# dangeross/rust-bitcoinconsensus

Hardware: AMD Instinct MI355X
Metric: ECDSA verifies/sec (node) at 1/2/4/8 MI355X; % of int-ALU roofline (higher is better)
Workload: dtype u32; 1 GPU; C2: synthetic P2WPKH inputs, BIP143 sighash + ECDSA verify (BASELINE.json configs[1]); inputs_per_gpu=1000000, global_inputs=1000000, parallelism=shard x1 (independent tuples, no collective)

## Files before the change

### rust-bitcoinconsensus_amd/csrc/ecdsa_lane.h

```cpp
#pragma once
#include "secp256k1_device.h"
#include "sha256_device.h"

namespace bcc {

#ifndef BCC_WQ_BITS
#define BCC_WQ_BITS 4
#endif
constexpr int WQ = BCC_WQ_BITS;
#ifndef BCC_WG_BITS
#define BCC_WG_BITS 10
#endif
constexpr int WG = BCC_WG_BITS;
constexpr int QTAB = 1 << (WQ - 1);
constexpr int GTAB = 1 << (WG - 1);
constexpr int TOPQ = (127 / WQ) * WQ;
static_assert(TOPQ + WQ >= 128, "top Q digit must cover bit 127");
constexpr int TOPG = (127 / WG) * WG;
static_assert(TOPG + WG >= 128 && TOPG <= TOPQ, "top G digit must cover bit 127 inside the ladder");

BCC_HD u32 bits_at(u32 l0, u32 l1, u32 l2, u32 l3, int pos, int w) {
    int li = pos >> 5, sh = pos & 31;
    u32 a = li == 0 ? l0 : li == 1 ? l1 : li == 2 ? l2 : l3;
    u32 b = li == 0 ? l1 : li == 1 ? l2 : li == 2 ? l3 : 0u;
    u32 v = sh ? ((a >> sh) | (b << (32 - sh))) : a;
    return v & ((1u << w) - 1u);
}

BCC_HD u32 digit_index(u32 l0, u32 l1, u32 l2, u32 l3, int pos, int w, int top, bool& neg) {
    u32 v = bits_at(l0, l1, l2, l3, pos + 1, w);
    if (pos == top) {
        neg = false;
        return v;
    }
    u32 half = 1u << (w - 1), mask = half - 1u;
    bool positive = (v & half) != 0;
    neg = !positive;
    return positive ? (v & mask) : (~v & mask);
}

struct QTableArray {
    fe e[QTAB][3];
    BCC_HD void put(int i, int f, const fe& a) { e[i][f] = a; }
    BCC_HD void get(int i, int f, fe& a) const { a = e[i][f]; }
    BCC_HD void get_pair(int i, int which, fe& x, fe& y) const {
        x = e[i][which];
        y = e[i][2];
    }
};

struct GTableArray {
    const fe* xy;
    BCC_HD void get(int tab, int i, fe& x, fe& y) const {
        x = xy[(tab * GTAB + i) * 2 + 0];
        y = xy[(tab * GTAB + i) * 2 + 1];
    }
};

BCC_HD void acc_add(gej& acc, bool& inf, const fe& px, const fe& py, const fe& sigma,
                    bool use_zinv) {
    if (inf) {
        if (use_zinv) {
            fe s2, s3;
            fe_sqr(s2, sigma);
            fe_mul(s3, s2, sigma);
            fe_mul(acc.x, px, s2);
            fe_mul(acc.y, py, s3);
        } else {
            acc.x = px;
            acc.y = py;
        }
        acc.z = fe_one();
        inf = false;
        return;
    }
    gej r;
    bool rinf;
    gej_add_zinv(r, rinf, acc, px, py, sigma, use_zinv);
    acc = r;
    inf = rinf;
}

enum : u32 {
    LS_VALID = 1u, LS_NEG0 = 2u, LS_NEG1 = 4u, LS_CORR0 = 8u,
};

template <class QT>
BCC_HD void build_q_table_coz(const fe& qx, const fe& qy, QT& qt, fe& sigma) {
    fe dx, dy, tx, ty;
    {
        fe b, e, l, sx, m, t;
        fe_sqr(b, qx);
        fe_sqr(e, qy);
        fe_sqr(l, e);
        fe_add(t, qx, e);
        fe_sqr(t, t);
        fe_sub(t, t, b);
        fe_sub(t, t, l);
        fe_shl<1>(sx, t);
        fe_shl<1>(m, b);
        fe_add(m, m, b);
        fe_sqr(t, m);
        fe_shl<1>(dx, sx);
        fe_sub(dx, t, dx);
        fe_sub(t, sx, dx);
        fe_mul(t, m, t);
        fe_shl<3>(ty, l);
        fe_sub(dy, t, ty);
        tx = sx;
    }
    qt.put(0, 0, tx);
    qt.put(0, 2, ty);
    for (int i = 1; i < QTAB; i++) {
        fe h, c, w1, w2, d, a1, t, ry;
        fe_sub(h, dx, tx);
        fe_sqr(c, h);
        fe_mul(w1, dx, c);
        fe_mul(w2, tx, c);
        fe_sub(ry, dy, ty);
        fe_sqr(d, ry);
        fe_sub(t, w1, w2);
        fe_mul(a1, dy, t);
        fe_sub(t, d, w1);
        fe_sub(tx, t, w2);
        fe_sub(t, w1, tx);
        fe_mul(t, ry, t);
        fe_sub(ty, t, a1);
        dx = w1;
        dy = a1;
        qt.put(i, 0, tx);
        qt.put(i, 2, ty);
        qt.put(i, 1, h);
    }
    fe f = fe_one(), f2, f3, beta;
    {
        const u32 bl[8] = BCC_BETA_LIMBS;
        fe_set(beta, bl);
    }
    for (int i = QTAB - 1; i >= 0; i--) {
        fe ex, ey, h;
        qt.get(i, 0, ex);
        qt.get(i, 2, ey);
        if (i > 0) qt.get(i, 1, h);
        if (i < QTAB - 1) {
            fe_sqr(f2, f);
            fe_mul(f3, f2, f);
            fe_mul(ex, ex, f2);
            fe_mul(ey, ey, f3);
        }
        fe bx;
        fe_mul(bx, ex, beta);
        qt.put(i, 0, ex);
        qt.put(i, 1, bx);
        qt.put(i, 2, ey);
        if (i > 0) fe_mul(f, f, h);
    }
    fe y2;
    fe_shl<1>(y2, qy);
    fe_mul(sigma, f, y2);
}

BCC_HD void curve_rhs(fe& r, const fe& x) {
    fe seven = fe_const(7, 0, 0, 0, 0, 0, 0, 0);
    fe_sqr(r, x);
    fe_mul(r, r, x);
    fe_add(r, r, seven);
}


BCC_HD void schnorr_challenge(sc& e, const fe& rx, const fe& px, const sc& m) {
    const u32 N[8] = BCC_N_LIMBS;
    u32 s[8] = {0x9cecba11u, 0x23925381u, 0x11679112u, 0xd1627e0fu,
                0x97c87550u, 0x003cc765u, 0x90f61164u, 0x33e9b66au};
    u32 w[16];
#pragma unroll
    for (int j = 0; j < 8; j++) {
        w[j] = rx.v[7 - j];
        w[8 + j] = px.v[7 - j];
    }
    sha256_compress(s, w);
#pragma unroll
    for (int j = 0; j < 8; j++) w[j] = m.v[7 - j];
    w[8] = 0x80000000u;
#pragma unroll
    for (int j = 9; j < 15; j++) w[j] = 0;
    w[15] = 160 * 8;
    sha256_compress(s, w);
#pragma unroll
    for (int i = 0; i < 8; i++) e.v[i] = s[7 - i];
    if (!u256_lt(e.v, N)) {
        u32 tmp[8];
        u256_sub(tmp, e.v, N);
        for (int i = 0; i < 8; i++) e.v[i] = tmp[i];
    }
}

BCC_HD bool schnorr_y_even(const fe& ye, const fe& zinv) {
    fe z2, z3, y;
    fe_sqr(z2, zinv);
    fe_mul(z3, z2, zinv);
    fe_mul(y, ye, z3);
    fe_normalize(y);
    return (y.v[0] & 1u) == 0;
}

template <class GT>
BCC_HD bool ecmult_gen_lane(const sc& k_in, fe& xo, fe& yo, const GT& gt) {
    if (sc_is_zero(k_in)) return false;
    u32 c0 = k_in.v[0], c1 = k_in.v[1], c2 = k_in.v[2], c3 = k_in.v[3];
    u32 d0 = k_in.v[4], d1 = k_in.v[5], d2 = k_in.v[6], d3 = k_in.v[7];
    bool corr2 = (c0 & 1u) == 0, corr3 = (d0 & 1u) == 0;
    c0 |= 1u;
    d0 |= 1u;
    fe one = fe_one();
    gej acc;
    bool inf = false;
    {
        bool ng;
        u32 idx = digit_index(c0, c1, c2, c3, TOPG, WG, TOPG, ng);
        gt.get(0, (int)idx, acc.x, acc.y);
        acc.z = one;
    }
    for (int pos = TOPG; pos >= 0; pos--) {
        if (pos != TOPG && !inf) {
            gej t;
            gej_double(t, acc);
            acc = t;
        }
        if (pos % WG) continue;
        for (int slot = 2; slot < 4; slot++) {
            if (slot == 2 && pos == TOPG) continue;
            bool dneg;
            u32 idx = slot == 2 ? digit_index(c0, c1, c2, c3, pos, WG, TOPG, dneg)
                                : digit_index(d0, d1, d2, d3, pos, WG, TOPG, dneg);
            fe px, py;
            gt.get(slot - 2, (int)idx, px, py);
            if (dneg) fe_neg(py, py);
// ... 117 lines not shown
```

### rust-bitcoinconsensus_amd/csrc/ecdsa_twist.h

```cpp
#pragma once
#include <stddef.h>

#include <algorithm>
#include <thread>
#include <vector>

#include "ecdsa_lane.h"

namespace bcc {

#ifndef BCC_COMB_BITS
#define BCC_COMB_BITS 16
#endif
constexpr int WC = BCC_COMB_BITS;
constexpr int CTAB = 1 << (WC - 1);
constexpr int CTOP = (256 + WC - 1) / WC - 1;
constexpr int CWIN = CTOP + 1;
static_assert(WC * CTOP + 1 + (WC - 1) >= 256, "top comb digit must cover bit 255");

enum : u32 {
    LS_NEGU1 = 1u << 7,
    LS_U1ZERO = 1u << 8,
    LS_COMP = 1u << 9,
    LS_PAR = 1u << 10,
// ... 69 lines not shown
    build_q_table_coz(qx, qy, qt, st.sigma);
    st.flags = flags;
    return true;
}

BCC_HD bool twist_prep_u2(u32 flags, const sc& r_in, const sc& s_in, const sc* sinv_pre,
                          TwistState& st, sc* sinv_out = nullptr) {
    const u32 N[8] = BCC_N_LIMBS;
    st.flags = 0;
    if (!(flags & LS_VALID)) return false;
    if (u256_is_zero(r_in.v) || u256_is_zero(s_in.v)) return false;
    if (!u256_lt(r_in.v, N) || !u256_lt(s_in.v, N)) return false;
    sc sinv, u2, k1, k2;
    if (sinv_pre) sinv = *sinv_pre;
    else sc_inv(sinv, s_in);
    if (sinv_out) *sinv_out = sinv;
    sc_mul(u2, r_in, sinv);
    sc_split_lambda(k1, k2, u2);
    if ((k1.v[4] | k1.v[5] | k1.v[6] | k1.v[7]) != 0) {
        sc_neg(k1, k1);
        flags |= LS_NEG0;
    }
    if ((k2.v[4] | k2.v[5] | k2.v[6] | k2.v[7]) != 0) {
        sc_neg(k2, k2);
        flags |= LS_NEG1;
    }
    for (int i = 0; i < 4; i++) {
        st.k[0][i] = k1.v[i];
        st.k[1][i] = k2.v[i];
    }
    for (int s = 0; s < 2; s++) {
        if ((st.k[s][0] & 1u) == 0) flags |= LS_CORR0 << s;
        st.k[s][0] |= 1u;
    }
    st.flags = flags;
    st.r = r_in;
    return true;
}

BCC_HD void twist_prep_u1(const sc& m_in, const sc& sinv, u32* flags, u32 (&k2)[4], u32 (&k3)[4]) {
    const u32 N[8] = BCC_N_LIMBS;
    sc m = m_in, u1;
    if (!u256_lt(m.v, N)) {
        u32 tmp[8];
        u256_sub(tmp, m.v, N);
        for (int i = 0; i < 8; i++) m.v[i] = tmp[i];
    }
    sc_mul(u1, m, sinv);
    if (sc_is_zero(u1)) {
        *flags |= LS_U1ZERO;
        u1.v[0] = 1u;
    } else if ((u1.v[0] & 1u) == 0) {
        sc_neg(u1, u1);
        *flags |= LS_NEGU1;
    }
    for (int i = 0; i < 4; i++) {
        k2[i] = u1.v[i];
        k3[i] = u1.v[4 + i];
    }
}

BCC_HD bool twist_prep_scalars(u32 flags, const sc& r_in, const sc& s_in, const sc& m_in,
                               const sc* sinv_pre, TwistState& st) {
    sc sinv;
    if (!twist_prep_u2(flags, r_in, s_in, sinv_pre, st, &sinv)) return false;
    twist_prep_u1(m_in, sinv, &st.flags, st.k[2], st.k[3]);
    return true;
}

template <class QT>
BCC_HD bool twist_prep_lane(u32 tag, const fe& px, const fe& py, const sc& r_in, const sc& s_in,
                            const sc& m_in, const sc* sinv_pre, QT& qt, TwistState& st) {
    if (!twist_prep_key(tag, px, py, qt, st)) return false;
    return twist_prep_scalars(st.flags, r_in, s_in, m_in, sinv_pre, st);
}

template <class ST, class QT>
BCC_HD bool twist_accumulate_q(const ST& st, const QT& qt, gej& acc) {
    const bool neg0 = (st.flags & LS_NEG0) != 0, neg1 = (st.flags & LS_NEG1) != 0;
    const fe one = fe_one();
    bool inf = false;
    {
        bool ng;
        u32 idx = digit_index(st.kword(0, 0), st.kword(0, 1), st.kword(0, 2), st.kword(0, 3), TOPQ,
                              WQ, TOPQ, ng);
        qt.get((int)idx, 0, acc.x);
        qt.get((int)idx, 2, acc.y);
        if (neg0) fe_neg(acc.y, acc.y);
        acc.z = one;
    }
#pragma unroll 1
    for (int pos = TOPQ; pos >= -1; pos--) {
        if (pos >= 0 && pos != TOPQ && !inf) {
            gej t;
            gej_double(t, acc);
            acc = t;
        }
        if (pos >= 0 && (pos % WQ) != 0) continue;
#pragma unroll 1
        for (int slot = 0; slot < 2; slot++) {
            const bool kneg = slot == 0 ? neg0 : neg1;
            u32 idx;
            bool sneg;
            if (pos >= 0) {
                if (slot == 0 && pos == TOPQ) continue;
                bool dneg;
                idx = digit_index(st.kword(slot, 0), st.kword(slot, 1), st.kword(slot, 2),
                                  st.kword(slot, 3), pos, WQ, TOPQ, dneg);
                sneg = dneg ^ kneg;
            } else {
                if (!(st.flags & (LS_CORR0 << slot))) continue;
                idx = 0;
                sneg = !kneg;
            }
            fe px, py;
            qt.get_pair((int)idx, slot, px, py);
            if (sneg) fe_neg(py, py);
            acc_add(acc, inf, px, py, one, false);
        }
    }
    return inf;
}

template <class ST, class QT>
BCC_HD bool twist_accumulate_q_half(const ST& st, const QT& qt, gej& acc, int slot) {
    const bool kneg = (st.flags & (slot == 0 ? LS_NEG0 : LS_NEG1)) != 0;
    const fe one = fe_one();
    bool inf = false;
    {
        bool ng;
        const u32 idx = digit_index(st.kword(slot, 0), st.kword(slot, 1), st.kword(slot, 2),
                                    st.kword(slot, 3), TOPQ, WQ, TOPQ, ng);
        qt.get_pair((int)idx, slot, acc.x, acc.y);
        if (kneg) fe_neg(acc.y, acc.y);
        acc.z = one;
    }
#pragma unroll 1
    for (int pos = TOPQ; pos >= -1; pos--) {
        if (pos >= 0 && pos != TOPQ && !inf) {
            gej t;
            gej_double(t, acc);
            acc = t;
        }
        if (pos >= 0 && ((pos % WQ) != 0 || pos == TOPQ)) continue;
        u32 idx;
        bool sneg;
        if (pos >= 0) {
            bool dneg;
            idx = digit_index(st.kword(slot, 0), st.kword(slot, 1), st.kword(slot, 2),
                              st.kword(slot, 3), pos, WQ, TOPQ, dneg);
            sneg = dneg ^ kneg;
        } else {
            if (!(st.flags & (LS_CORR0 << slot))) continue;
            idx = 0;
            sneg = !kneg;
        }
        fe px, py;
        qt.get_pair((int)idx, slot, px, py);
        if (sneg) fe_neg(py, py);
        acc_add(acc, inf, px, py, one, false);
    }
    return inf;
}

template <class ST, class GC>
BCC_HD bool twist_accumulate_g(const ST& st, const GC& gc, gej& acc) {
    const fe one = fe_one();
    bool inf = false;
    {
        bool ng;
        u32 idx = comb_digit(st, WC * CTOP, ng);
        gc.get(CTOP, (int)idx, acc.x, acc.y);
        acc.z = one;
    }
#pragma unroll 1
    for (int win = CTOP - 1; win >= 0; win--) {
        bool neg;
        u32 idx = comb_digit(st, WC * win, neg);
        fe px, py;
        gc.get(win, (int)idx, px, py);
        if (neg) fe_neg(py, py);
        acc_add(acc, inf, px, py, one, false);
    }
    if (st.flags & LS_NEGU1) fe_neg(acc.y, acc.y);
    if (st.flags & LS_U1ZERO) inf = true;
    return inf;
}

BCC_HD bool twist_combine(const gej& A, const gej& B, const fe& sigma, const fe& v, const sc& r,
                          fe& al, fe& be, fe& K) {
    fe zb, zb2, z12, u1, u2, s1, s2, h, hh, t;
    fe_mul(zb, B.z, sigma);
    fe_sqr(zb2, zb);
    fe_sqr(z12, A.z);
    fe_mul(u2, B.x, z12);
    fe_mul(t, z12, A.z);
    fe_mul(s2, B.y, t);
    fe_mul(t, A.y, zb2);
    fe_mul(t, t, zb);
    fe_mul(s1, t, v);
    fe_mul(t, A.x, zb2);
    fe_mul(u1, t, v);
    fe_sub(h, u2, u1);
    if (fe_is_zero(h)) return false;
    fe_mul(be, s2, s1);
    fe_shl<1>(be, be);
    if (fe_is_zero(be)) return false;
    fe_sqr(hh, h);
    fe_mul(t, z12, zb2);
    fe_mul(t, t, v);
    fe_mul(K, t, hh);
    fe xr;
    for (int i = 0; i < 8; i++) xr.v[i] = r.v[i];
    fe_mul(al, xr, K);
    fe_sqr(t, s2);
    fe_sub(al, al, t);
    fe_sqr(t, s1);
    fe_mul(t, t, v);
    fe_sub(al, al, t);
    fe_mul(t, hh, h);
    fe_add(al, al, t);
    fe_mul(t, u1, hh);
    fe_shl<1>(t, t);
    fe_add(al, al, t);
    return true;
}

BCC_HD bool twist_is_key_y(const fe& al, const fe& binv, const fe& v, const fe& ychk, u32 flags) {
    fe g, g2;
    fe_mul(g, al, binv);
    fe_neg(g, g);
    fe_normalize(g);
    fe_sqr(g2, g);
    if (!fe_equal(g2, v)) return false;
    if (flags & LS_COMP) return (g.v[0] & 1u) == ((flags & LS_PAR) ? 1u : 0u);
    return fe_equal(g, ychk);
}

BCC_HD int twist_final(const fe& al, const fe& K, const fe& binv, const fe& v, const fe& ychk,
                       u32 flags, const sc& r) {
    if (twist_is_key_y(al, binv, v, ychk, flags)) return 1;
    const u32 PMN[8] = BCC_PMN_LIMBS;
    if (!u256_lt(r.v, PMN)) return 0;
    const u32 N[8] = BCC_N_LIMBS;
    fe nf, t, al2;
    fe_set(nf, N);
    fe_mul(t, K, nf);
    fe_add(al2, al, t);
    return twist_is_key_y(al2, binv, v, ychk, flags) ? 1 : 0;
}

BCC_HD void gej_add_gej(gej& r, bool& inf, const gej& a, const gej& b) {
    fe z22, z12, u1, u2, s1, s2, h, rr, hh, hhh, v, t;
    fe_sqr(z22, b.z);
    fe_sqr(z12, a.z);
    fe_mul(u1, a.x, z22);
    fe_mul(u2, b.x, z12);
    fe_mul(s1, a.y, z22);
    fe_mul(s1, s1, b.z);
    fe_mul(s2, b.y, z12);
    fe_mul(s2, s2, a.z);
    fe_sub(h, u2, u1);
    fe_sub(rr, s2, s1);
    if (fe_is_zero(h)) {
        if (fe_is_zero(rr)) {
            gej_double(r, a);
            inf = false;
        } else {
            inf = true;
            r = a;
        }
        return;
    }
    fe_sqr(hh, h);
    fe_mul(hhh, h, hh);
    fe_mul(v, u1, hh);
    fe_mul(t, a.z, b.z);
    fe_mul(r.z, t, h);
    fe_sqr(t, rr);
    fe_sub(t, t, hhh);
    fe_sub(t, t, v);
    fe_sub(r.x, t, v);
    fe_sub(t, v, r.x);
    fe_mul(t, rr, t);
    fe_mul(hhh, s1, hhh);
    fe_sub(r.y, t, hhh);
    inf = false;
}

BCC_HD int twist_exceptional(const gej& A, bool ainf, const gej& B, bool binf, const fe& sigma,
                             const fe& v, const fe& ychk, u32 flags, const sc& r) {
    const u32 N[8] = BCC_N_LIMBS;
    fe w;
    if (flags & LS_COMP) {
        if (!fe_sqrt(w, v)) return 0;
        fe_normalize(w);
        if ((w.v[0] & 1u) != ((flags & LS_PAR) ? 1u : 0u)) fe_neg(w, w);
    } else {
        w = ychk;
    }
    if (ainf && binf) return 0;
    gej be = B, R;
    bool rinf = false;
    fe zb;
    fe_mul(zb, B.z, sigma);
    fe_mul(be.z, zb, w);
    if (binf) R = A;
    else if (ainf) R = be;
    else gej_add_gej(R, rinf, A, be);
    if (rinf) return 0;
    fe z2, lhs, xr;
    fe_sqr(z2, R.z);
    for (int i = 0; i < 8; i++) xr.v[i] = r.v[i];
    fe_mul(lhs, xr, z2);
    if (fe_equal(lhs, R.x)) return 1;
    const u32 PMN[8] = BCC_PMN_LIMBS;
    if (!u256_lt(r.v, PMN)) return 0;
    u32 xn[8];
    u256_add(xn, r.v, N);
    for (int i = 0; i < 8; i++) xr.v[i] = xn[i];
    fe_mul(lhs, xr, z2);
    return fe_equal(lhs, R.x) ? 1 : 0;
}

enum : u32 { TW_REJECT = 0, TW_NORMAL = 1, TW_EXCEPT = 2 };

template <class QT, class GC>
BCC_HD int ecdsa_verify_twist_lane(u32 tag, const fe& px, const fe& py, const sc& r,
                                   const sc& s, const sc& m, QT& qt, const GC& gc) {
    TwistState st;
    if (!twist_prep_lane(tag, px, py, r, s, m, nullptr, qt, st)) return 0;
    gej A, B;
    const bool binf = twist_accumulate_q(st, qt, B);
    const bool ainf = twist_accumulate_g(st, gc, A);
    fe al, be, K;
    if (binf || ainf || !twist_combine(A, B, st.sigma, st.v, st.r, al, be, K))
        return twist_exceptional(A, ainf, B, binf, st.sigma, st.v, st.ychk, st.flags, st.r);
    fe binv;
    fe_inv(binv, be);
    return twist_final(al, K, binv, st.v, st.ychk, st.flags, st.r);
}

#if !defined(__HIP_DEVICE_COMPILE__)
inline int wnaf5_128(int8_t (&d)[132], const u32 (&k)[4]) {
    typedef unsigned __int128 u128;
    u128 lo = (u128)((uint64_t)k[2] | (uint64_t)k[3] << 32) << 64 | ((uint64_t)k[0] | (uint64_t)k[1] << 32);
    uint64_t hi = 0;
    int n = 0;
    while (lo | hi) {
        int v = 0;
        if (lo & 1) {
            v = (int)(lo & 31);
            if (v >= 16) v -= 32;
            if (v > 0) {
                lo -= (u128)v;
            } else {
                const u128 o = lo;
                lo += (u128)(-v);
                if (lo < o) hi++;
            }
        }
        d[n++] = (int8_t)v;
        lo = lo >> 1 | (u128)(hi & 1) << 127;
        hi >>= 1;
    }
    return n;
}

template <class ST, class QT>
inline bool twist_accumulate_q_wnaf(const ST& st, const u32 (&k1)[4], const u32 (&k2)[4], const QT& qt,
                                    gej& acc) {
    int8_t d[2][132];
    const int n0 = wnaf5_128(d[0], k1), n1 = wnaf5_128(d[1], k2);
    const bool kneg[2] = {(st.flags & LS_NEG0) != 0, (st.flags & LS_NEG1) != 0};
    const fe one = fe_one();
    bool inf = true;
    acc.x = acc.y = fe_zero();
    acc.z = one;
    for (int i = std::max(n0, n1) - 1; i >= 0; i--) {
        if (!inf) {
            gej t;
            gej_double(t, acc);
            acc = t;
        }
        for (int slot = 0; slot < 2; slot++) {
            const int v = i < (slot ? n1 : n0) ? d[slot][i] : 0;
            if (v == 0) continue;
            fe px, py;
            qt.get_pair((v < 0 ? -v : v) >> 1, slot, px, py);
            if ((v < 0) != kneg[slot]) fe_neg(py, py);
            acc_add(acc, inf, px, py, one, false);
        }
    }
    return inf;
}

template <class QT, class GC>
inline int ecdsa_verify_twist_host(u32 tag, const fe& px, const fe& py, const sc& r, const sc& s,
                                   const sc& m, QT& qt, const GC& gc) {
    TwistState st;
    if (!twist_prep_key(tag, px, py, qt, st)) return 0;
    sc sinv;
    if (!twist_prep_u2(st.flags, r, s, nullptr, st, &sinv)) return 0;
    u32 k1[4], k2[4];
    for (int i = 0; i < 4; i++) {
        k1[i] = st.k[0][i];
        k2[i] = st.k[1][i];
    }
    if (st.flags & LS_CORR0) k1[0] &= ~1u;
    if (st.flags & (LS_CORR0 << 1)) k2[0] &= ~1u;
    twist_prep_u1(m, sinv, &st.flags, st.k[2], st.k[3]);
    gej A, B;
    const bool binf = twist_accumulate_q_wnaf(st, k1, k2, qt, B);
    const bool ainf = twist_accumulate_g(st, gc, A);
    fe al, be, K;
    if (binf || ainf || !twist_combine(A, B, st.sigma, st.v, st.r, al, be, K))
        return twist_exceptional(A, ainf, B, binf, st.sigma, st.v, st.ychk, st.flags, st.r);
    fe binv;
    fe_inv(binv, be);
    return twist_final(al, K, binv, st.v, st.ychk, st.flags, st.r);
}
#endif


template <class QT>
BCC_HD bool schnorr_twist_prep(const fe& px, const fe& rx, const sc& s_in, const sc& m, QT& qt,
                               TwistState& st) {
    const u32 N[8] = BCC_N_LIMBS;
    st.flags = 0;
    if (!fe_lt_p(rx)) return false;
    if (!u256_lt(s_in.v, N)) return false;
    if (!fe_lt_p(px)) return false;
    fe v;
    curve_rhs(v, px);
    sc e, u2, u1 = s_in, k1, k2;
    schnorr_challenge(e, rx, px, m);
    sc_neg(u2, e);
    u32 flags = LS_VALID | LS_COMP;
    sc_split_lambda(k1, k2, u2);
    if ((k1.v[4] | k1.v[5] | k1.v[6] | k1.v[7]) != 0) {
        sc_neg(k1, k1);
        flags |= LS_NEG0;
    }
    if ((k2.v[4] | k2.v[5] | k2.v[6] | k2.v[7]) != 0) {
        sc_neg(k2, k2);
        flags |= LS_NEG1;
    }
    if (sc_is_zero(u1)) {
        flags |= LS_U1ZERO;
        u1.v[0] = 1u;
    } else if ((u1.v[0] & 1u) == 0) {
        sc_neg(u1, u1);
        flags |= LS_NEGU1;
    }
    for (int i = 0; i < 4; i++) {
        st.k[0][i] = k1.v[i];
        st.k[1][i] = k2.v[i];
        st.k[2][i] = u1.v[i];
        st.k[3][i] = u1.v[4 + i];
    }
    for (int q = 0; q < 2; q++) {
        if ((st.k[q][0] & 1u) == 0) flags |= LS_CORR0 << q;
        st.k[q][0] |= 1u;
    }
    st.flags = flags;
    for (int i = 0; i < 8; i++) st.r.v[i] = rx.v[i];
    st.v = v;
    st.ychk = fe_zero();
    fe qx, qy;
    fe_mul(qx, px, v);
    fe_sqr(qy, v);
    build_q_table_coz(qx, qy, qt, st.sigma);
    return true;
}

BCC_HD bool schnorr_twist_combine(const gej& A, const gej& B, const fe& sigma, const fe& v,
                                  const fe& rx, fe& al, fe& be, fe& dd, fe& c0, fe& c1) {
    fe zb, zb2, z12, u1, u2, s1, s2, h, hh, t, x3r, m;
    fe_mul(zb, B.z, sigma);
    fe_sqr(zb2, zb);
    fe_sqr(z12, A.z);
    fe_mul(u2, B.x, z12);
    fe_mul(t, z12, A.z);
    fe_mul(s2, B.y, t);
    fe_mul(t, A.y, zb2);
    fe_mul(t, t, zb);
    fe_mul(s1, t, v);
    fe_mul(t, A.x, zb2);
    fe_mul(u1, t, v);
    fe_sub(h, u2, u1);
    if (fe_is_zero(h)) return false;
    fe_mul(be, s2, s1);
    fe_shl<1>(be, be);
    if (fe_is_zero(be)) return false;
    fe_mul(t, A.z, zb);
    fe_mul(t, t, h);
    fe_sqr(dd, t);
// ... 155 lines not shown
```

### rust-bitcoinconsensus_amd/csrc/ecdsa_verify.hip

```cpp
#include <atomic>
#include <cstdio>
#include <cstdlib>
#include <memory>
#include <string>

#include "bcc_amd.h"
#include "ecdsa_lane.h"
#include "ecdsa_twist.h"
#include "gpu_common.h"
#include "host/devices.h"
#include "host/host_verify.h"
#include "host/taproot_host.h"
#include "pipeline.h"

namespace bcc {

constexpr size_t LANE_STRIDE = 64;
__device__ __forceinline__ u32* lane_words(u32* base, size_t t, int W) {
    return base + (t >> 6) * (size_t)(W * 64) + (t & 63);
}
__device__ __forceinline__ const u32* lane_words(const u32* base, size_t t, int W) {
    return base + (t >> 6) * (size_t)(W * 64) + (t & 63);
}

struct QTableGlobal {
    u32* base;
    __device__ static int field_off(int f) { return f == 0 ? 0 : f == 1 ? 16 : 8; }
    __device__ void put(int i, int f, const fe& a) {
        uint4* p = reinterpret_cast<uint4*>(base + i * 32 + field_off(f));
        p[0] = make_uint4(a.v[0], a.v[1], a.v[2], a.v[3]);
        p[1] = make_uint4(a.v[4], a.v[5], a.v[6], a.v[7]);
        if (f == 2) {
            uint4* q = reinterpret_cast<uint4*>(base + i * 32 + 24);
            q[0] = p[0];
            q[1] = p[1];
        }
    }
    __device__ void get(int i, int f, fe& a) const {
        const uint4* p = reinterpret_cast<const uint4*>(base + i * 32 + field_off(f));
        const uint4 u = p[0], v = p[1];
        a.v[0] = u.x; a.v[1] = u.y; a.v[2] = u.z; a.v[3] = u.w;
        a.v[4] = v.x; a.v[5] = v.y; a.v[6] = v.z; a.v[7] = v.w;
    }
    __device__ void get_pair(int i, int which, fe& x, fe& y) const {
        const uint4* p = reinterpret_cast<const uint4*>(base + i * 32 + 16 * which);
        const uint4 a = p[0], b = p[1], c = p[2], d = p[3];
        x.v[0] = a.x; x.v[1] = a.y; x.v[2] = a.z; x.v[3] = a.w;
        x.v[4] = b.x; x.v[5] = b.y; x.v[6] = b.z; x.v[7] = b.w;
        y.v[0] = c.x; y.v[1] = c.y; y.v[2] = c.z; y.v[3] = c.w;
        y.v[4] = d.x; y.v[5] = d.y; y.v[6] = d.z; y.v[7] = d.w;
    }
};
__device__ __forceinline__ u32* lane_table(u32* qtab, size_t t);
constexpr int QTABLE_WORDS = QTAB * 32;
__device__ __forceinline__ u32* lane_table(u32* qtab, size_t t) { return qtab + t * QTABLE_WORDS; }
constexpr int PRE_WORDS = 8;

__device__ __forceinline__ void load_be32(fe& r, const uint8_t* p) {
    const uint4* q = reinterpret_cast<const uint4*>(p);
    uint4 a = q[0], b = q[1];
    u32 w[8] = {a.x, a.y, a.z, a.w, b.x, b.y, b.z, b.w};
    fe_from_be_words(r, w);
}
__device__ __forceinline__ void load_be32(sc& r, const uint8_t* p) {
    fe t;
    load_be32(t, p);
#pragma unroll
    for (int k = 0; k < 8; k++) r.v[k] = t.v[k];
}
__device__ __forceinline__ void load_limbs(sc& r, const u32* p) {
    const uint4* q = reinterpret_cast<const uint4*>(p);
    uint4 a = q[0], b = q[1];
    r.v[0] = a.x; r.v[1] = a.y; r.v[2] = a.z; r.v[3] = a.w;
    r.v[4] = b.x; r.v[5] = b.y; r.v[6] = b.z; r.v[7] = b.w;
}
__device__ __forceinline__ void store_limbs(u32* p, const sc& a) {
    uint4* q = reinterpret_cast<uint4*>(p);
    q[0] = make_uint4(a.v[0], a.v[1], a.v[2], a.v[3]);
    q[1] = make_uint4(a.v[4], a.v[5], a.v[6], a.v[7]);
}

__device__ __forceinline__ void sanitize_s(sc& s) {
    const u32 N[8] = BCC_N_LIMBS;
    if (u256_is_zero(s.v) || !u256_lt(s.v, N)) {
        s.v[0] = 1;
#pragma unroll
        for (int k = 1; k < 8; k++) s.v[k] = 0;
    }
}

#ifndef BCC_INV_PER_THREAD
#define BCC_INV_PER_THREAD 16
#endif
#ifndef BCC_FIN_PER_THREAD
#define BCC_FIN_PER_THREAD 16
#endif
constexpr size_t INV_PER_THREAD = BCC_INV_PER_THREAD;
constexpr size_t FIN_PER_THREAD = BCC_FIN_PER_THREAD;

__global__ __launch_bounds__(256) void batch_sinv_kernel(const uint8_t* __restrict__ ps,
                                                         u32* __restrict__ sinv, size_t n,
                                                         size_t T) {
    const size_t t = (size_t)blockIdx.x * blockDim.x + threadIdx.x;
    if (t >= n || t >= T) return;
    sc acc, s;
    size_t last = t;
    load_be32(acc, ps + 32 * t);
    sanitize_s(acc);
    store_limbs(sinv + 8 * t, acc);
    for (size_t i = t + T; i < n; i += T) {
        load_be32(s, ps + 32 * i);
        sanitize_s(s);
        sc_mul(acc, acc, s);
        store_limbs(sinv + 8 * i, acc);
        last = i;
    }
    sc inv;
    sc_inv(inv, acc);
    for (size_t i = last; i >= t + T; i -= T) {
        load_be32(s, ps + 32 * i);
        sanitize_s(s);
        sc prev, out;
        load_limbs(prev, sinv + 8 * (i - T));
        sc_mul(out, inv, prev);
        sc_mul(inv, inv, s);
        store_limbs(sinv + 8 * i, out);
    }
    store_limbs(sinv + 8 * t, inv);
}
// ... 44 lines not shown
};

struct GCombGlobal {
    const u32* base;
    __device__ void get(int win, int i, fe& x, fe& y) const {
        const uint4* q = reinterpret_cast<const uint4*>(base + ((size_t)win * CTAB + i) * 16);
        const uint4 a = q[0], b = q[1], c = q[2], d = q[3];
        x.v[0] = a.x; x.v[1] = a.y; x.v[2] = a.z; x.v[3] = a.w;
        x.v[4] = b.x; x.v[5] = b.y; x.v[6] = b.z; x.v[7] = b.w;
        y.v[0] = c.x; y.v[1] = c.y; y.v[2] = c.z; y.v[3] = c.w;
        y.v[4] = d.x; y.v[5] = d.y; y.v[6] = d.z; y.v[7] = d.w;
    }
};

__device__ __forceinline__ void park_gej(u32* q, const gej& a, bool inf) {
    uint4* p = reinterpret_cast<uint4*>(q);
    p[0] = make_uint4(a.x.v[0], a.x.v[1], a.x.v[2], a.x.v[3]);
    p[1] = make_uint4(a.x.v[4], a.x.v[5], a.x.v[6], a.x.v[7]);
    p[2] = make_uint4(a.y.v[0], a.y.v[1], a.y.v[2], a.y.v[3]);
    p[3] = make_uint4(a.y.v[4], a.y.v[5], a.y.v[6], a.y.v[7]);
    p[4] = make_uint4(a.z.v[0], a.z.v[1], a.z.v[2], a.z.v[3]);
    p[5] = make_uint4(a.z.v[4], a.z.v[5], a.z.v[6], a.z.v[7]);
    p[6] = make_uint4(inf ? 1u : 0u, 0u, 0u, 0u);
}
__device__ __forceinline__ bool unpark_gej(const u32* q, gej& a) {
    asm volatile("" : "+v"(q));
    const uint4* p = reinterpret_cast<const uint4*>(q);
    uint4 u;
    u = p[0]; a.x.v[0] = u.x; a.x.v[1] = u.y; a.x.v[2] = u.z; a.x.v[3] = u.w;
    u = p[1]; a.x.v[4] = u.x; a.x.v[5] = u.y; a.x.v[6] = u.z; a.x.v[7] = u.w;
    u = p[2]; a.y.v[0] = u.x; a.y.v[1] = u.y; a.y.v[2] = u.z; a.y.v[3] = u.w;
    u = p[3]; a.y.v[4] = u.x; a.y.v[5] = u.y; a.y.v[6] = u.z; a.y.v[7] = u.w;
    u = p[4]; a.z.v[0] = u.x; a.z.v[1] = u.y; a.z.v[2] = u.z; a.z.v[3] = u.w;
    u = p[5]; a.z.v[4] = u.x; a.z.v[5] = u.y; a.z.v[6] = u.z; a.z.v[7] = u.w;
    return p[6].x != 0;
}
constexpr int PARK_B = 0, PARK_A = 32;

__global__ __launch_bounds__(256) __attribute__((amdgpu_waves_per_eu(3, 3))) void ecdsa_tprep_kernel(
    const uint8_t* __restrict__ tag, const uint8_t* __restrict__ px,
    const uint8_t* __restrict__ py, const uint8_t* __restrict__ pr, const uint8_t* __restrict__ ps,
    const uint8_t* __restrict__ pm, const u32* __restrict__ psinv, size_t base, size_t cnt,
    u32* __restrict__ qtab, u32* __restrict__ state) {
    const size_t t = (size_t)blockIdx.x * blockDim.x + threadIdx.x;
    if (t >= cnt) return;
    const size_t i = base + t;
    fe x, y;
    sc r, s, m, si;
    load_be32(x, px + 32 * i);
    load_be32(y, py + 32 * i);
    load_be32(r, pr + 32 * i);
    load_be32(s, ps + 32 * i);
    load_be32(m, pm + 32 * i);
    load_limbs(si, psinv + 8 * i);
    QTableGlobal qt{lane_table(qtab, t)};
    TwistState st;
    twist_prep_lane(tag[i], x, y, r, s, m, &si, qt, st);
    u32* w = lane_words(state, t, TSTATE_WORDS);
#pragma unroll
    for (int a = 0; a < 4; a++)
#pragma unroll
        for (int b = 0; b < 4; b++) w[(T_K + a * 4 + b) * LANE_STRIDE] = st.k[a][b];
    w[T_FLAGS * LANE_STRIDE] = st.flags;
    tw_store(w, T_SIGMA, st.sigma.v);
    tw_store(w, T_R, st.r.v);
    tw_store(w, T_V, st.v.v);
    tw_store(w, T_Y, st.ychk.v);
}

#ifndef BCC_TLADDER_WG
#define BCC_TLADDER_WG 256
#endif
constexpr int TLADDER_WG = BCC_TLADDER_WG;

__device__ __forceinline__ void twist_q_part(u32* lt, const TwistStateView& st) {
    gej B;
    const bool binf = twist_accumulate_q(st, QTableGlobal{lt}, B);
    park_gej(lt + PARK_B, B, binf);
}

template <bool BIP340>
__device__ __forceinline__ void twist_g_part(u32* w, u32* lt, const u32* gcomb, TwistStateView& st) {
    u32 stat = TW_NORMAL;
    gej A, B;
    const bool ainf = twist_accumulate_g(st, GCombGlobal{gcomb}, A);
    const bool binf = unpark_gej(lt + PARK_B, B);
    fe v, al, be, K;
    sc r;
    st.get_v(v);
    st.get_r(r);
    bool ok;
    if constexpr (BIP340) {
        fe c0, c1, rx;
#pragma unroll
        for (int j = 0; j < 8; j++) rx.v[j] = r.v[j];
        ok = !binf && !ainf && schnorr_twist_combine(A, B, st.sigma, v, rx, al, be, K, c0, c1);
        if (ok) {
            tw_store(w, T_C0, c0.v);
            tw_store(w, T_C1, c1.v);
        }
    } else {
        ok = !binf && !ainf && twist_combine(A, B, st.sigma, v, r, al, be, K);
    }
    if (!ok) {
        park_gej(lt + PARK_A, A, ainf);
        stat = TW_EXCEPT;
    } else {
        tw_store(w, T_AL, al.v);
        tw_store(w, T_BE, be.v);
        tw_store(w, T_KK, K.v);
    }
    w[T_STAT * LANE_STRIDE] = stat;
}

template <bool BIP340>
__global__ __launch_bounds__(TLADDER_WG) __attribute__((amdgpu_waves_per_eu(BCC_LADDER_WAVES, BCC_LADDER_WAVES))) void twist_ladder_kernel(
    u32* __restrict__ state, u32* __restrict__ qtab, const u32* __restrict__ gcomb, size_t cnt) {
    const size_t t = (size_t)blockIdx.x * blockDim.x + threadIdx.x;
    if (t >= cnt) return;
    u32* w = lane_words(state, t, TSTATE_WORDS);
    TwistStateView st;
    st.p = w;
    st.flags = w[T_FLAGS * LANE_STRIDE];
    if (!(st.flags & LS_VALID)) {
        w[T_STAT * LANE_STRIDE] = TW_REJECT;
        return;
    }
    tw_load(st.sigma.v, w, T_SIGMA);
    u32* lt = lane_table(qtab, t);
    twist_q_part(lt, st);
    twist_g_part<BIP340>(w, lt, gcomb, st);
}

__global__ __launch_bounds__(TLADDER_WG) __attribute__((amdgpu_waves_per_eu(BCC_LADDER_WAVES, BCC_LADDER_WAVES))) void schnorr_tladder_kernel(
    const uint8_t* __restrict__ psig, const uint8_t* __restrict__ pm,
    const uint8_t* __restrict__ ppk, size_t base, size_t cnt, u32* __restrict__ qtab,
    u32* __restrict__ state, const u32* __restrict__ gcomb) {
    const size_t t = (size_t)blockIdx.x * blockDim.x + threadIdx.x;
    if (t >= cnt) return;
    const size_t i = base + t;
    u32* w = lane_words(state, t, TSTATE_WORDS);
    u32* lt = lane_table(qtab, t);
    {
        fe px, rx;
        sc s, m;
        load_be32(rx, psig + 64 * i);
        load_be32(s, psig + 64 * i + 32);
        load_be32(m, pm + 32 * i);
        load_be32(px, ppk + 32 * i);
        QTableGlobal qt{lt};
        TwistState st;
        schnorr_twist_prep(px, rx, s, m, qt, st);
#pragma unroll
        for (int a = 0; a < 4; a++)
#pragma unroll
            for (int b = 0; b < 4; b++) w[(T_K + a * 4 + b) * LANE_STRIDE] = st.k[a][b];
        w[T_FLAGS * LANE_STRIDE] = st.flags;
        tw_store(w, T_SIGMA, st.sigma.v);
        tw_store(w, T_R, st.r.v);
        tw_store(w, T_V, st.v.v);
        tw_store(w, T_Y, st.ychk.v);
    }
    TwistStateView sv;
    sv.p = w;
    sv.flags = w[T_FLAGS * LANE_STRIDE];
    if (!(sv.flags & LS_VALID)) {
        w[T_STAT * LANE_STRIDE] = TW_REJECT;
        return;
    }
    tw_load(sv.sigma.v, w, T_SIGMA);
    twist_q_part(lt, sv);
    twist_g_part<true>(w, lt, gcomb, sv);
}

#ifndef BCC_LADDERQ_WAVES
#define BCC_LADDERQ_WAVES BCC_LADDER_WAVES
#endif
__global__ __launch_bounds__(TLADDER_WG) __attribute__((amdgpu_waves_per_eu(BCC_LADDERQ_WAVES, BCC_LADDERQ_WAVES))) void twist_keyq_kernel(
    const uint8_t* __restrict__ tag, const uint8_t* __restrict__ px, const uint8_t* __restrict__ py,
    const uint8_t* __restrict__ pr, const uint8_t* __restrict__ ps, const u32* __restrict__ psinv,
    size_t cnt, u32* __restrict__ qtab, u32* __restrict__ state, const u32* __restrict__ emap,
    size_t ecount, size_t base) {
    const size_t t = base + (size_t)blockIdx.x * blockDim.x + threadIdx.x;
    if (t >= cnt) return;
    if (emap && emap[t] < ecount) return;
    u32* w = lane_words(state, t, TSTATE_WORDS);
    u32* lt = lane_table(qtab, t);
    {
// ... 828 lines not shown
```

### rust-bitcoinconsensus_amd/csrc/secp256k1_device.h

```cpp
#pragma once
#include <stdint.h>
#include <string.h>

#if defined(__HIPCC__)
#include <hip/hip_runtime.h>
#include "fe_asm.h"
#include "fe_asm_gen.h"
#define BCC_HD __host__ __device__ __attribute__((always_inline)) inline
#define BCC_HD_NOINLINE __host__ __device__ __attribute__((noinline))
#else
#define BCC_HD inline
#define BCC_HD_NOINLINE
#endif

#include "modinv_device.h"

namespace bcc {

typedef uint32_t u32;
typedef uint64_t u64;

struct fe {
    u32 v[8];
};
// ... 697 lines not shown
    {
        const u32 a[8] = BCC_MB1_LIMBS, b[8] = BCC_MB2_LIMBS, l[8] = BCC_LAMBDA_LIMBS;
#pragma unroll
        for (int i = 0; i < 8; i++) {
            mb1.v[i] = a[i];
            mb2.v[i] = b[i];
            lam.v[i] = l[i];
        }
    }
    sc_mul_shift_384(c1, k, G1);
    sc_mul_shift_384(c2, k, G2);
    sc_mul(c1, c1, mb1);
    sc_mul(c2, c2, mb2);
    sc_add(k2, c1, c2);
    sc_mul(k1, k2, lam);
    sc_neg(k1, k1);
    sc_add(k1, k1, k);
}

struct gej {
    fe x, y, z;
};

BCC_HD void gej_double(gej& r, const gej& a) {
    fe A, B, C, D, E, F, t;
    fe_sqr(A, a.x);
    fe_sqr(B, a.y);
    fe_sqr(C, B);
    fe_add(t, a.x, B);
    fe_sqr(t, t);
    fe_sub(t, t, A);
    fe_sub(t, t, C);
    fe_shl<1>(D, t);
    fe_shl<1>(E, A);
    fe_add(E, E, A);
    fe_sqr(F, E);
    fe_mul(r.z, a.y, a.z);
    fe_shl<1>(r.z, r.z);
    fe_shl<1>(t, D);
    fe_sub(r.x, F, t);
    fe_sub(t, D, r.x);
    fe_mul(t, E, t);
    fe_shl<3>(C, C);
    fe_sub(r.y, t, C);
}

BCC_HD void gej_add_zinv(gej& r, bool& inf, const gej& a, const fe& bx, const fe& by,
                         const fe& bzinv, bool use_zinv, fe* hout = nullptr) {
    fe az, z12, u2, s2, h, rr, hh, hhh, v, t;
    if (use_zinv) fe_mul(az, a.z, bzinv);
    else az = a.z;
    fe_sqr(z12, az);
    fe_mul(u2, bx, z12);
    fe_mul(s2, by, z12);
    fe_mul(s2, s2, az);
    fe_sub(h, u2, a.x);
    fe_sub(rr, s2, a.y);
    if (fe_is_zero(h)) {
        if (fe_is_zero(rr)) {
            gej_double(r, a);
            inf = false;
        } else {
            inf = true;
            r = a;
        }
        return;
    }
    if (hout) *hout = h;
    fe_sqr(hh, h);
    fe_mul(hhh, h, hh);
    fe_mul(v, a.x, hh);
    fe_mul(r.z, a.z, h);
    fe_sqr(t, rr);
    fe_sub(t, t, hhh);
    fe_sub(t, t, v);
    fe_sub(r.x, t, v);
    fe_sub(t, v, r.x);
    fe_mul(t, rr, t);
    fe_mul(hhh, a.y, hhh);
    fe_sub(r.y, t, hhh);
    inf = false;
}

}
```

Baseline: 115.1 million verifies/s.

## Use XYZZ coordinates for G comb, precompute negated Q-table y, merge first adds

The generator comb accumulation moves from Jacobian to XYZZ coordinates, so each mixed add needs fewer squarings and the final combine reuses ZZ and ZZZ directly. The Q table now stores a negated y entry, so lookups pick the sign by address instead of calling fe_neg on the loaded value. The first two digits of both ladders are merged with a cheaper affine plus affine add, which skips one generic add and one doubling iteration. In exchange each point carries an extra field element, which raises register pressure and state size, and the exceptional path pays a conversion back to Jacobian.

```diff
diff --git a/rust-bitcoinconsensus_amd/csrc/ecdsa_lane.h b/rust-bitcoinconsensus_amd/csrc/ecdsa_lane.h
--- a/rust-bitcoinconsensus_amd/csrc/ecdsa_lane.h
+++ b/rust-bitcoinconsensus_amd/csrc/ecdsa_lane.h
@@ -40,12 +40,12 @@
 }
 
 struct QTableArray {
-    fe e[QTAB][3];
+    fe e[QTAB][4];
     BCC_HD void put(int i, int f, const fe& a) { e[i][f] = a; }
     BCC_HD void get(int i, int f, fe& a) const { a = e[i][f]; }
-    BCC_HD void get_pair(int i, int which, fe& x, fe& y) const {
+    BCC_HD void get_pair(int i, int which, bool neg, fe& x, fe& y) const {
         x = e[i][which];
-        y = e[i][2];
+        y = e[i][neg ? 3 : 2];
     }
 };
 
@@ -77,6 +77,22 @@
     gej r;
     bool rinf;
     gej_add_zinv(r, rinf, acc, px, py, sigma, use_zinv);
+    acc = r;
+    inf = rinf;
+}
+
+BCC_HD void acc_add_xz(gexz& acc, bool& inf, const fe& px, const fe& py) {
+    if (inf) {
+        acc.x = px;
+        acc.y = py;
+        acc.zz = fe_one();
+        acc.zzz = fe_one();
+        inf = false;
+        return;
+    }
+    gexz r;
+    bool rinf;
+    gexz_add_ge(r, rinf, acc, px, py);
     acc = r;
     inf = rinf;
 }
@@ -148,11 +164,13 @@
             fe_mul(ex, ex, f2);
             fe_mul(ey, ey, f3);
         }
-        fe bx;
+        fe bx, ny;
         fe_mul(bx, ex, beta);
+        fe_neg(ny, ey);
         qt.put(i, 0, ex);
         qt.put(i, 1, bx);
         qt.put(i, 2, ey);
+        qt.put(i, 3, ny);
         if (i > 0) fe_mul(f, f, h);
     }
     fe y2;
diff --git a/rust-bitcoinconsensus_amd/csrc/ecdsa_twist.h b/rust-bitcoinconsensus_amd/csrc/ecdsa_twist.h
--- a/rust-bitcoinconsensus_amd/csrc/ecdsa_twist.h
+++ b/rust-bitcoinconsensus_amd/csrc/ecdsa_twist.h
@@ -175,16 +175,18 @@
     bool inf = false;
     {
         bool ng;
+        fe ax, ay, bx, by;
         u32 idx = digit_index(st.kword(0, 0), st.kword(0, 1), st.kword(0, 2), st.kword(0, 3), TOPQ,
                               WQ, TOPQ, ng);
-        qt.get((int)idx, 0, acc.x);
-        qt.get((int)idx, 2, acc.y);
-        if (neg0) fe_neg(acc.y, acc.y);
-        acc.z = one;
+        qt.get_pair((int)idx, 0, neg0, ax, ay);
+        idx = digit_index(st.kword(1, 0), st.kword(1, 1), st.kword(1, 2), st.kword(1, 3), TOPQ, WQ,
+                          TOPQ, ng);
+        qt.get_pair((int)idx, 1, neg1, bx, by);
+        gej_add_affine(acc, inf, ax, ay, bx, by);
     }
 #pragma unroll 1
-    for (int pos = TOPQ; pos >= -1; pos--) {
-        if (pos >= 0 && pos != TOPQ && !inf) {
+    for (int pos = TOPQ - 1; pos >= -1; pos--) {
+        if (pos >= 0 && !inf) {
             gej t;
             gej_double(t, acc);
             acc = t;
@@ -196,7 +198,6 @@
             u32 idx;
             bool sneg;
             if (pos >= 0) {
-                if (slot == 0 && pos == TOPQ) continue;
                 bool dneg;
                 idx = digit_index(st.kword(slot, 0), st.kword(slot, 1), st.kword(slot, 2),
                                   st.kword(slot, 3), pos, WQ, TOPQ, dneg);
@@ -207,8 +208,7 @@
                 sneg = !kneg;
             }
             fe px, py;
-            qt.get_pair((int)idx, slot, px, py);
-            if (sneg) fe_neg(py, py);
+            qt.get_pair((int)idx, slot, sneg, px, py);
             acc_add(acc, inf, px, py, one, false);
         }
     }
@@ -224,8 +224,7 @@
         bool ng;
         const u32 idx = digit_index(st.kword(slot, 0), st.kword(slot, 1), st.kword(slot, 2),
                                     st.kword(slot, 3), TOPQ, WQ, TOPQ, ng);
-        qt.get_pair((int)idx, slot, acc.x, acc.y);
-        if (kneg) fe_neg(acc.y, acc.y);
+        qt.get_pair((int)idx, slot, kneg, acc.x, acc.y);
         acc.z = one;
     }
 #pragma unroll 1
@@ -249,8 +248,7 @@
             sneg = !kneg;
         }
         fe px, py;
-        qt.get_pair((int)idx, slot, px, py);
-        if (sneg) fe_neg(py, py);
+        qt.get_pair((int)idx, slot, sneg, px, py);
         acc_add(acc, inf, px, py, one, false);
     }
     return inf;
@@ -261,13 +259,17 @@
     const fe one = fe_one();
     bool inf = false;
     {
-        bool ng;
+        bool ng, neg;
+        fe ax, ay, bx, by;
         u32 idx = comb_digit(st, WC * CTOP, ng);
-        gc.get(CTOP, (int)idx, acc.x, acc.y);
-        acc.z = one;
+        gc.get(CTOP, (int)idx, ax, ay);
+        idx = comb_digit(st, WC * (CTOP - 1), neg);
+        gc.get(CTOP - 1, (int)idx, bx, by);
+        if (neg) fe_neg(by, by);
+        gej_add_affine(acc, inf, ax, ay, bx, by);
     }
 #pragma unroll 1
-    for (int win = CTOP - 1; win >= 0; win--) {
+    for (int win = CTOP - 2; win >= 0; win--) {
         bool neg;
         u32 idx = comb_digit(st, WC * win, neg);
         fe px, py;
@@ -280,15 +282,41 @@
     return inf;
 }
 
-BCC_HD bool twist_combine(const gej& A, const gej& B, const fe& sigma, const fe& v, const sc& r,
+template <class ST, class GC>
+BCC_HD bool twist_accumulate_g_xz(const ST& st, const GC& gc, gexz& acc) {
+    bool inf = false;
+    {
+        bool ng, neg;
+        fe ax, ay, bx, by;
+        u32 idx = comb_digit(st, WC * CTOP, ng);
+        gc.get(CTOP, (int)idx, ax, ay);
+        idx = comb_digit(st, WC * (CTOP - 1), neg);
+        gc.get(CTOP - 1, (int)idx, bx, by);
+        if (neg) fe_neg(by, by);
+        gexz_add_affine(acc, inf, ax, ay, bx, by);
+    }
+#pragma unroll 1
+    for (int win = CTOP - 2; win >= 0; win--) {
+        bool neg;
+        u32 idx = comb_digit(st, WC * win, neg);
+        fe px, py;
+        gc.get(win, (int)idx, px, py);
+        if (neg) fe_neg(py, py);
+        acc_add_xz(acc, inf, px, py);
+    }
+    if (st.flags & LS_NEGU1) fe_neg(acc.y, acc.y);
+    if (st.flags & LS_U1ZERO) inf = true;
+    return inf;
+}
+
+BCC_HD bool twist_combine(const gexz& A, const gej& B, const fe& sigma, const fe& v, const sc& r,
                           fe& al, fe& be, fe& K) {
-    fe zb, zb2, z12, u1, u2, s1, s2, h, hh, t;
+    fe zb, zb2, u1, u2, s1, s2, h, hh, t;
+    const fe& z12 = A.zz;
     fe_mul(zb, B.z, sigma);
     fe_sqr(zb2, zb);
-    fe_sqr(z12, A.z);
     fe_mul(u2, B.x, z12);
-    fe_mul(t, z12, A.z);
-    fe_mul(s2, B.y, t);
+    fe_mul(s2, B.y, A.zzz);
     fe_mul(t, A.y, zb2);
     fe_mul(t, t, zb);
     fe_mul(s1, t, v);
@@ -416,6 +444,13 @@
     return fe_equal(lhs, R.x) ? 1 : 0;
 }
 
+BCC_HD int twist_exceptional(const gexz& A, bool ainf, const gej& B, bool binf, const fe& sigma,
+                             const fe& v, const fe& ychk, u32 flags, const sc& r) {
+    gej a;
+    gexz_to_gej(a, A);
+    return twist_exceptional(a, ainf, B, binf, sigma, v, ychk, flags, r);
+}
+
 enum : u32 { TW_REJECT = 0, TW_NORMAL = 1, TW_EXCEPT = 2 };
 
 template <class QT, class GC>
@@ -423,9 +458,10 @@
                                    const sc& s, const sc& m, QT& qt, const GC& gc) {
     TwistState st;
     if (!twist_prep_lane(tag, px, py, r, s, m, nullptr, qt, st)) return 0;
-    gej A, B;
+    gexz A;
+    gej B;
     const bool binf = twist_accumulate_q(st, qt, B);
-    const bool ainf = twist_accumulate_g(st, gc, A);
+    const bool ainf = twist_accumulate_g_xz(st, gc, A);
     fe al, be, K;
     if (binf || ainf || !twist_combine(A, B, st.sigma, st.v, st.r, al, be, K))
         return twist_exceptional(A, ainf, B, binf, st.sigma, st.v, st.ychk, st.flags, st.r);
@@ -480,8 +516,7 @@
             const int v = i < (slot ? n1 : n0) ? d[slot][i] : 0;
             if (v == 0) continue;
             fe px, py;
-            qt.get_pair((v < 0 ? -v : v) >> 1, slot, px, py);
-            if ((v < 0) != kneg[slot]) fe_neg(py, py);
+            qt.get_pair((v < 0 ? -v : v) >> 1, slot, (v < 0) != kneg[slot], px, py);
             acc_add(acc, inf, px, py, one, false);
         }
     }
@@ -503,9 +538,10 @@
     if (st.flags & LS_CORR0) k1[0] &= ~1u;
     if (st.flags & (LS_CORR0 << 1)) k2[0] &= ~1u;
     twist_prep_u1(m, sinv, &st.flags, st.k[2], st.k[3]);
-    gej A, B;
+    gexz A;
+    gej B;
     const bool binf = twist_accumulate_q_wnaf(st, k1, k2, qt, B);
-    const bool ainf = twist_accumulate_g(st, gc, A);
+    const bool ainf = twist_accumulate_g_xz(st, gc, A);
     fe al, be, K;
     if (binf || ainf || !twist_combine(A, B, st.sigma, st.v, st.r, al, be, K))
         return twist_exceptional(A, ainf, B, binf, st.sigma, st.v, st.ychk, st.flags, st.r);
diff --git a/rust-bitcoinconsensus_amd/csrc/ecdsa_verify.hip b/rust-bitcoinconsensus_amd/csrc/ecdsa_verify.hip
--- a/rust-bitcoinconsensus_amd/csrc/ecdsa_verify.hip
+++ b/rust-bitcoinconsensus_amd/csrc/ecdsa_verify.hip
@@ -3,6 +3,7 @@
 #include <cstdlib>
 #include <memory>
 #include <string>
+#include <type_traits>
 
 #include "bcc_amd.h"
 #include "ecdsa_lane.h"
@@ -25,16 +26,11 @@
 
 struct QTableGlobal {
     u32* base;
-    __device__ static int field_off(int f) { return f == 0 ? 0 : f == 1 ? 16 : 8; }
+    __device__ static int field_off(int f) { return f == 0 ? 0 : f == 1 ? 16 : f == 2 ? 8 : 24; }
     __device__ void put(int i, int f, const fe& a) {
         uint4* p = reinterpret_cast<uint4*>(base + i * 32 + field_off(f));
         p[0] = make_uint4(a.v[0], a.v[1], a.v[2], a.v[3]);
         p[1] = make_uint4(a.v[4], a.v[5], a.v[6], a.v[7]);
-        if (f == 2) {
-            uint4* q = reinterpret_cast<uint4*>(base + i * 32 + 24);
-            q[0] = p[0];
-            q[1] = p[1];
-        }
     }
     __device__ void get(int i, int f, fe& a) const {
         const uint4* p = reinterpret_cast<const uint4*>(base + i * 32 + field_off(f));
@@ -42,9 +38,10 @@
         a.v[0] = u.x; a.v[1] = u.y; a.v[2] = u.z; a.v[3] = u.w;
         a.v[4] = v.x; a.v[5] = v.y; a.v[6] = v.z; a.v[7] = v.w;
     }
-    __device__ void get_pair(int i, int which, fe& x, fe& y) const {
+    __device__ void get_pair(int i, int which, bool neg, fe& x, fe& y) const {
         const uint4* p = reinterpret_cast<const uint4*>(base + i * 32 + 16 * which);
-        const uint4 a = p[0], b = p[1], c = p[2], d = p[3];
+        const uint4* q = reinterpret_cast<const uint4*>(base + i * 32 + (neg ? 24 : 8));
+        const uint4 a = p[0], b = p[1], c = q[0], d = q[1];
         x.v[0] = a.x; x.v[1] = a.y; x.v[2] = a.z; x.v[3] = a.w;
         x.v[4] = b.x; x.v[5] = b.y; x.v[6] = b.z; x.v[7] = b.w;
         y.v[0] = c.x; y.v[1] = c.y; y.v[2] = c.z; y.v[3] = c.w;
@@ -255,8 +252,11 @@
 template <bool BIP340>
 __device__ __forceinline__ void twist_g_part(u32* w, u32* lt, const u32* gcomb, TwistStateView& st) {
     u32 stat = TW_NORMAL;
-    gej A, B;
-    const bool ainf = twist_accumulate_g(st, GCombGlobal{gcomb}, A);
+    typename std::conditional<BIP340, gej, gexz>::type A;
+    gej B;
+    bool ainf;
+    if constexpr (BIP340) ainf = twist_accumulate_g(st, GCombGlobal{gcomb}, A);
+    else ainf = twist_accumulate_g_xz(st, GCombGlobal{gcomb}, A);
     const bool binf = unpark_gej(lt + PARK_B, B);
     fe v, al, be, K;
     sc r;
@@ -276,7 +276,13 @@
         ok = !binf && !ainf && twist_combine(A, B, st.sigma, v, r, al, be, K);
     }
     if (!ok) {
-        park_gej(lt + PARK_A, A, ainf);
+        if constexpr (BIP340) {
+            park_gej(lt + PARK_A, A, ainf);
+        } else {
+            gej a;
+            gexz_to_gej(a, A);
+            park_gej(lt + PARK_A, a, ainf);
+        }
         stat = TW_EXCEPT;
     } else {
         tw_store(w, T_AL, al.v);
diff --git a/rust-bitcoinconsensus_amd/csrc/secp256k1_device.h b/rust-bitcoinconsensus_amd/csrc/secp256k1_device.h
--- a/rust-bitcoinconsensus_amd/csrc/secp256k1_device.h
+++ b/rust-bitcoinconsensus_amd/csrc/secp256k1_device.h
@@ -803,4 +803,127 @@
     inf = false;
 }
 
-}
+BCC_HD void gej_add_affine(gej& r, bool& inf, const fe& ax, const fe& ay, const fe& bx,
+                           const fe& by) {
+    fe h, rr, hh, hhh, v, t;
+    fe_sub(h, bx, ax);
+    fe_sub(rr, by, ay);
+    if (fe_is_zero(h)) {
+        gej a;
+        a.x = ax;
+        a.y = ay;
+        a.z = fe_one();
+        if (fe_is_zero(rr)) {
+            gej_double(r, a);
+            inf = false;
+        } else {
+            inf = true;
+            r = a;
+        }
+        return;
+    }
+    fe_sqr(hh, h);
+    fe_mul(hhh, h, hh);
+    fe_mul(v, ax, hh);
+    r.z = h;
+    fe_sqr(t, rr);
+    fe_sub(t, t, hhh);
+    fe_sub(t, t, v);
+    fe_sub(r.x, t, v);
+    fe_sub(t, v, r.x);
+    fe_mul(t, rr, t);
+    fe_mul(hhh, ay, hhh);
+    fe_sub(r.y, t, hhh);
+    inf = false;
+}
+
+struct gexz {
+    fe x, y, zz, zzz;
+};
+
+BCC_HD void gexz_to_gej(gej& r, const gexz& a) {
+    fe z2, z3;
+    fe_sqr(z2, a.zz);
+    fe_mul(z3, z2, a.zz);
+    fe_mul(r.x, a.x, z2);
+    fe_mul(r.y, a.y, z3);
+    r.z = a.zzz;
+}
+
+BCC_HD void gexz_from_gej(gexz& r, const gej& a) {
+    r.x = a.x;
+    r.y = a.y;
+    fe_sqr(r.zz, a.z);
+    fe_mul(r.zzz, r.zz, a.z);
+}
+
+BCC_HD void gexz_add_affine(gexz& r, bool& inf, const fe& ax, const fe& ay, const fe& bx,
+                            const fe& by) {
+    fe h, rr, v, t;
+    fe_sub(h, bx, ax);
+    fe_sub(rr, by, ay);
+    if (fe_is_zero(h)) {
+        gej a, d;
+        a.x = ax;
+        a.y = ay;
+        a.z = fe_one();
+        if (fe_is_zero(rr)) {
+            gej_double(d, a);
+            gexz_from_gej(r, d);
+            inf = false;
+        } else {
+            inf = true;
+            gexz_from_gej(r, a);
+        }
+        return;
+    }
+    fe_sqr(r.zz, h);
+    fe_mul(r.zzz, h, r.zz);
+    fe_mul(v, ax, r.zz);
+    fe_sqr(t, rr);
+    fe_sub(t, t, r.zzz);
+    fe_sub(t, t, v);
+    fe_sub(r.x, t, v);
+    fe_sub(t, v, r.x);
+    fe_mul(t, rr, t);
+    fe_mul(v, ay, r.zzz);
+    fe_sub(r.y, t, v);
+    inf = false;
+}
+
+BCC_HD void gexz_add_ge(gexz& r, bool& inf, const gexz& a, const fe& bx, const fe& by) {
+    fe u2, s2, h, rr, hh, hhh, v, t;
+    fe_mul(u2, bx, a.zz);
+    fe_mul(s2, by, a.zzz);
+    fe_sub(h, u2, a.x);
+    fe_sub(rr, s2, a.y);
+    if (fe_is_zero(h)) {
+        if (fe_is_zero(rr)) {
+            gej j, d;
+            gexz_to_gej(j, a);
+            gej_double(d, j);
+            gexz_from_gej(r, d);
+            inf = false;
+        } else {
+            inf = true;
+            r = a;
+        }
+        return;
+    }
+    fe_sqr(hh, h);
+    fe_mul(hhh, h, hh);
+    fe_mul(v, a.x, hh);
+    fe_mul(r.zz, a.zz, hh);
+    fe_mul(r.zzz, a.zzz, hhh);
+    fe_sqr(t, rr);
+    fe_sub(t, t, hhh);
+    fe_sub(t, t, v);
+    fe_sub(r.x, t, v);
+    fe_sub(t, v, r.x);
+    fe_mul(t, rr, t);
+    fe_mul(hhh, a.y, hhh);
+    fe_sub(r.y, t, hhh);
+    inf = false;
+}
+
+}
```

New measurement: 117.3 million verifies/s, median of 6. 1.9% higher.
